# usnistgov/semantic-segmentation-unet

Hardware: AMD Instinct MI355X
Metric: training images/sec (higher is better)
Workload: dtype f32; 1 GPU; U-Net train step, synthetic 512x512x1, 2 classes, batch 8/GPU, f32 (BASELINE config 2); global_batch=8, parallelism=dp1, measured=2/bf16x6: 236.5 img/s

## Files before the change

include/unet_hip.h:

```cpp
#ifndef UNET_HIP_H
#define UNET_HIP_H
#include <stddef.h>
#include <stdint.h>
#ifdef __cplusplus
extern "C" {
#endif

#define UNET_OK 0
#define UNET_EINVAL (-1)
#define UNET_ENOSPC (-2)

#define UNET_HIP_ABI_VERSION 9
int unet_hip_abi_version(void);

int unet_conv3x3_mfma_supported(int Cin, int Cout);
int unet_conv3x3_fwd_mfma(const float* x, int ldx, const float* w, const float* bias, float* out, int ldo,
                          int N, int H, int W, int Cin, int Cout, int relu, void* stream);
int unet_conv3x3_dgrad_mfma(const float* dz, int lddz, const float* w, float* dx, int lddx,
                            int N, int H, int W, int Cin, int Cout, void* stream);
size_t unet_conv3x3_wgrad_mfma_workspace(int N, int H, int W, int Cin, int Cout);
int unet_conv3x3_wgrad_mfma(const float* xin, int ldx, const float* dz, int lddz, float* dw,
                            int N, int H, int W, int Cin, int Cout, void* ws, size_t ws_bytes, void* stream);
int unet_winograd_weight_transform(const float* w, float* U, int Cin, int Cout, int mode, void* stream);
int unet_winograd_weight_transform_batch(const void* jobs, int njobs, int total_blocks, void* stream);
// ... 81 lines not shown
int unet_convT2x2_wgrad_x6(const float* xin, int ldx, const float* dz, int lddz, float* dw,
                           int N, int H, int W, int Cin, int Cout, void* ws, size_t ws_bytes, void* stream);
size_t unet_convT2x2_wgrad_workspace(int N, int H, int W, int Cin, int Cout);
int unet_convT2x2_wgrad(const float* xin, int ldx, const float* dz, int lddz, float* dw,
                        int N, int H, int W, int Cin, int Cout, void* ws, size_t ws_bytes, void* stream);

int unet_bf16_pack_weights_batch(const void* jobs, int njobs, int total_blocks, void* stream);
int unet_convT2x2_bf16_supported(int N, int H, int W, int Cin, int Cout);
size_t unet_convT2x2_bf16_packed_bytes(int Cin, int Cout);
int unet_convT2x2_bf16_pack_weights(const float* w, void* packed, int Cin, int Cout, int mode, void* stream);
int unet_convT2x2_bf16_stats_rows(int N, int H, int W, int Cin, int Cout, int dgrad);
int unet_convT2x2_fwd_bf16(const void* x, int ldx, int x_bf16, const void* wp, const float* bias, void* out, int ldo, int out_bf16,
                           int N, int H, int W, int Cin, int Cout, float* stat_part, size_t stat_bytes, void* stream);
int unet_convT2x2_dgrad_bf16(const void* dz, int lddz, int dz_bf16, const void* wpd, void* dx, int lddx, int dx_bf16,
                             int N, int H, int W, int Cin, int Cout, const void* r_prev, int ldr, int r_bf16,
                             float* stat_part, size_t stat_bytes, void* stream);
int unet_convT2x2_wgrad_bf16_supported(int N, int H, int W, int Cin, int Cout);
size_t unet_convT2x2_wgrad_bf16_workspace(int N, int H, int W, int Cin, int Cout);
int unet_convT2x2_wgrad_bf16(const void* xin, int ldx, int x_bf16, const void* dz, int lddz, int dz_bf16, float* dw,
                                int N, int H, int W, int Cin, int Cout, void* ws, size_t ws_bytes, void* stream);

size_t unet_bn_workspace(long P, int C);
int unet_bn_train_stats(const float* r, int ldr, long P, int C, const float* gamma, const float* beta,
                        float eps, float momentum, int unbiased_moving_var, float* moving_mean, float* moving_var,
                        float* mean, float* invstd, float* scale, float* shift, void* ws, size_t ws_bytes, void* stream);
int unet_bn_train_finalize_partials(const float* part, int rows, long P, int C, const float* gamma, const float* beta,
                                    float eps, float momentum, int unbiased_moving_var, float* moving_mean, float* moving_var,
                                    float* mean, float* invstd, float* scale, float* shift, void* stream);
int unet_bn_eval_coeffs(const float* gamma, const float* beta, const float* moving_mean, const float* moving_var,
                        float eps, int C, float* scale, float* shift, void* stream);
int unet_bn_apply(const float* r, int ldr, const float* scale, const float* shift, float* y, int ldy, long P, int C, void* stream);
int unet_bn_apply_maxpool(const float* r, int ldr, const float* scale, const float* shift, float* y, int ldy,
                          float* pooled, int ldp, uint8_t* idx, int N, int H, int W, int C, void* stream);
int unet_bn_bwd(const float* dy, int lddy, const float* r, int ldr, const float* gamma, const float* mean,
                const float* invstd, long P, int C, int relu, float* dz, int lddz, float* dgamma, float* dbeta,
                float* dbias, void* ws, size_t ws_bytes, void* stream);

int unet_bn_bwd_pooled(const float* dy_skip, int lddy, const float* pooled_dy, int ldp, const uint8_t* idx, int N, int H, int W,
                       const float* r, int ldr, const float* gamma, const float* mean, const float* invstd, int C, int relu,
                       float* dz, int lddz, float* dgamma, float* dbeta, float* dbias, void* ws, size_t ws_bytes, void* stream);
int unet_bn_bwd_any(const void* dy, int lddy, const void* pooled_dy, int ldp, const uint8_t* idx, int N, int H, int W,
                    const void* r, int ldr, const float* gamma, const float* mean, const float* invstd, int C, int relu,
                    void* dz, int lddz, int dz_bf16, float* dgamma, float* dbeta, float* dbias, const float* part_sums, int rows,
                    void* ws, size_t ws_bytes, void* stream, int r_bf16, int dy_bf16, int pooled_dy_bf16, int* host_bias_rows);
int unet_bn_bwd_bias(const void* ws, int rows, int C, float* dbias, void* stream);
int unet_bn_apply_any(const void* r, int ldr, int r_bf16, const float* scale, const float* shift, void* y, int ldy, int y_bf16,
                      void* pooled, int ldp, uint8_t* idx, int N, int H, int W, int C, void* stream);
int unet_bn_finalize_apply_any(const float* part, int rows, const float* gamma, const float* beta, float eps, float momentum,
                               int unbiased_moving_var, float* moving_mean, float* moving_var, float* mean, float* invstd,
                               uint32_t* counter, uint32_t counter_target,
                               const void* r, int ldr, int r_bf16, float* scale, float* shift, void* y, int ldy, int y_bf16,
                               void* pooled, int ldp, uint8_t* idx, int N, int H, int W, int C, void* stream);
int unet_bn_bwd_from_partials(const float* dy, int lddy, const float* r, int ldr, const float* gamma, const float* mean,
                              const float* invstd, long P, int C, int relu, float* dz, int lddz, float* dgamma, float* dbeta,
                              float* dbias, const float* part_sums, int rows, void* ws, size_t ws_bytes, void* stream);

int unet_maxpool2x2_fwd(const void* x, int ldx, void* y, int ldy, uint8_t* idx, int N, int H, int W, int C, int t_bf16, void* stream);
int unet_maxpool2x2_bwd(const void* dy, int lddy, const uint8_t* idx, void* dx, int lddx,
                        int N, int H, int W, int C, int accumulate, int t_bf16, void* stream);
int unet_dropout(const void* x, int ldx, void* out, int ldo, long P, int C, const uint8_t* mask,
                 uint32_t seed, float rate, int t_bf16, void* stream);

size_t unet_softmax_ce_workspace(long P);
int unet_softmax_ce(const float* logits, int ldz, const int* labels_onehot, float* prob, float* dlogits, int lddz,
                    long P, int K, float label_smoothing, float loss_scale, float grad_scale, float ce_clip_eps,
                    float* loss_out, float* correct_out, void* ws, size_t ws_bytes, void* stream);
// ... 70 lines not shown
```

semantic-segmentation-unet_amd/csrc/norm.hip:

```cpp
#include "common.h"
#include <stdlib.h>

namespace {

typedef int i32x4v __attribute__((ext_vector_type(4)));
constexpr int kApplyNT = (UNET_NT & UNET_NT_LDAPPLY) != 0;

template <class T, int NT> __device__ __forceinline__ T bn_ld(const T* p) {
    if constexpr (NT != 0) return __builtin_nontemporal_load(p); else return *p;
}
template <int VEC, int NT = 0> __device__ __forceinline__ void vload(float (&v)[VEC], const float* p) {
    if constexpr (VEC == 8) {
        const f32x4 t = bn_ld<f32x4, NT>(reinterpret_cast<const f32x4*>(p)), u = bn_ld<f32x4, NT>(reinterpret_cast<const f32x4*>(p + 4));
        v[0] = t[0]; v[1] = t[1]; v[2] = t[2]; v[3] = t[3]; v[4] = u[0]; v[5] = u[1]; v[6] = u[2]; v[7] = u[3];
    } else if constexpr (VEC == 4) { const f32x4 t = bn_ld<f32x4, NT>(reinterpret_cast<const f32x4*>(p)); v[0] = t[0]; v[1] = t[1]; v[2] = t[2]; v[3] = t[3]; }
    else v[0] = *p;
}
__device__ __forceinline__ float bf_lo(unsigned w) { return __builtin_bit_cast(float, w << 16); }
__device__ __forceinline__ float bf_hi(unsigned w) { return __builtin_bit_cast(float, w & 0xffff0000u); }
template <int VEC, int NT = 0> __device__ __forceinline__ void vload_dt(float (&v)[VEC], const float* base, size_t idx, int in16) {
    if constexpr (VEC == 8) {
        if (in16) {
            const unet_u32x4 t = bn_ld<unet_u32x4, NT>(reinterpret_cast<const unet_u32x4*>(reinterpret_cast<const uint16_t*>(base) + idx));
            v[0] = bf_lo(t[0]); v[1] = bf_hi(t[0]); v[2] = bf_lo(t[1]); v[3] = bf_hi(t[1]);
// ... 282 lines not shown
        for (int e = 0; e < VEC; ++e) v[e] = fmaf(a[e], v[e], b[e]);
        vstore_dt<VEC>(y, (size_t)pix * ldy + c0, v, out16 & 1);
    }
}

template <int VEC>
__global__ __launch_bounds__(256) void bn_apply_pool_kernel(const float* __restrict__ r, int ldr, const float* scale,
        const float* shift, float* __restrict__ y, int ldy, float* __restrict__ pooled, int ldp, uint8_t* __restrict__ idx,
        int N, int H, int W, int C, int tpp, int out16, BnFin fin) {
    if (fin.part) bn_finalize_then_wait(fin, C, const_cast<float*>(scale), const_cast<float*>(shift));
    const Lay l = make_lay<VEC>(C, tpp);
    if (!l.active) return;
    const int H2 = H / 2, W2 = W / 2;
    const long total = (long)N * H2 * W2, S = (long)gridDim.x * l.npl;
    float a[VEC], b[VEC];
    bn_coef_load<VEC>(a, scale + l.c0, fin.part != nullptr); bn_coef_load<VEC>(b, shift + l.c0, fin.part != nullptr);
    for (long opix = (long)blockIdx.x * l.npl + l.pl; opix < total; opix += S) {
        long t = opix; const int ox = (int)(t % W2); t /= W2; const int oy = (int)(t % H2); const int n = (int)(t / H2);
        float best[VEC]; uint8_t bi[VEC];
        float v[4][VEC];
#pragma unroll
        for (int pos = 0; pos < 4; ++pos) {
            const size_t pix = (size_t)((long)n * H + 2 * oy + (pos >> 1)) * W + 2 * ox + (pos & 1);
            vload_dt<VEC, kApplyNT>(v[pos], r, pix * ldr + l.c0, out16 & 2);
        }
#pragma unroll
        for (int pos = 0; pos < 4; ++pos) {
            const size_t pix = (size_t)((long)n * H + 2 * oy + (pos >> 1)) * W + 2 * ox + (pos & 1);
#pragma unroll
            for (int e = 0; e < VEC; ++e) {
                v[pos][e] = fmaf(a[e], v[pos][e], b[e]);
                if (pos == 0 || v[pos][e] > best[e]) { best[e] = v[pos][e]; bi[e] = (uint8_t)pos; }
            }
            vstore_dt<VEC>(y, pix * ldy + l.c0, v[pos], out16 & 1);
        }
        vstore_dt<VEC>(pooled, (size_t)opix * ldp + l.c0, best, out16 & 1);
        const uint32_t w0 = (uint32_t)bi[0] | ((uint32_t)bi[1] << 8) | ((uint32_t)bi[2] << 16) | ((uint32_t)bi[3] << 24);
        if constexpr (VEC == 8) {
            const uint32_t w1 = (uint32_t)bi[4] | ((uint32_t)bi[5] << 8) | ((uint32_t)bi[6] << 16) | ((uint32_t)bi[7] << 24);
            *reinterpret_cast<uint2*>(idx + (size_t)opix * C + l.c0) = make_uint2(w0, w1);
        } else {
            *reinterpret_cast<uint32_t*>(idx + (size_t)opix * C + l.c0) = w0;
        }
    }
}

template <int VEC>
__global__ __launch_bounds__(256) void bn_bwd_reduce_kernel(const float* __restrict__ dy, int lddy, const float* __restrict__ r,
        int ldr, const float* __restrict__ mean, const float* __restrict__ invstd, long P, int C, int tpp, long ppb,
        double* __restrict__ part, PoolGrad pg, int dt) {
    extern __shared__ __attribute__((aligned(16))) double sRd[];
    const Lay l = make_lay<VEC>(C, tpp);
    const long p0 = (long)blockIdx.x * ppb; long p1 = p0 + ppb; if (p1 > P) p1 = P;
    double acc[2][VEC];
#pragma unroll
    for (int e = 0; e < VEC; ++e) { acc[0][e] = 0.0; acc[1][e] = 0.0; }
    if (l.active) {
        float mu[VEC]; vload<VEC>(mu, mean + l.c0);
        long pix = p0 + l.pl;
        const long st = l.npl;
        for (; pix + 3 * st < p1; pix += 4 * st) {
            float g[4][VEC], v[4][VEC];
#pragma unroll
            for (int u = 0; u < 4; ++u) {
                vload_dt<VEC>(g[u], dy, (size_t)(pix + u * st) * lddy + l.c0, dt & 4); vload_dt<VEC>(v[u], r, (size_t)(pix + u * st) * ldr + l.c0, dt & 2);
                add_pool_grad<VEC>(g[u], pg, pix + u * st, l.c0);
            }
// ... 445 lines not shown
    pl->vec = vec; pl->tpp = tpp; pl->nblk = (int)nblk; pl->ppb = (P + nblk - 1) / nblk;
    pl->smem2 = (size_t)256 * vec * 2 * sizeof(double); pl->smem1 = (size_t)256 * vec * sizeof(double);
    return true;
}

int nblk_for(long P) { (void)P; return (int)MAX_BLOCKS; }

constexpr bool bn_wide_always() { return true; }

int bn_cus() {
    static int cus = 0;
    if (!cus) { int dev = 0; hipDeviceProp_t pr; (void)hipGetDevice(&dev); cus = (hipGetDeviceProperties(&pr, dev) == hipSuccess && pr.multiProcessorCount > 0) ? pr.multiProcessorCount : 256; }
    return cus;
}

template <class K> int resident_grid(K kernel, size_t smem) {
    int per_cu = 0;
    if (hipOccupancyMaxActiveBlocksPerMultiprocessor(&per_cu, kernel, 256, smem) != hipSuccess || per_cu < 1) per_cu = 4;
    long g = (long)per_cu * bn_cus();
    return (int)(g > MAX_BLOCKS ? MAX_BLOCKS / bn_cus() * bn_cus() : g);
}
template <int VEC> int reduce_grid(size_t smem) { static int g = 0; if (!g) g = resident_grid(bn_bwd_reduce_kernel<VEC>, smem); return g; }
template <int VEC> int apply_grid(size_t smem) { static int g = 0; if (!g) g = resident_grid(bn_bwd_apply_kernel<VEC>, smem); return g; }
int pool16_grid(int which, size_t smem) {
    static int g[2] = {0, 0};
    if (!g[which]) g[which] = which ? resident_grid(bn_bwd_apply_pool16_kernel, smem) : resident_grid(bn_bwd_reduce_pool16_kernel, smem);
    return g[which];
}
int apply16_grid(size_t smem) { static int g = 0; if (!g) g = resident_grid(bn_bwd_apply16_kernel, smem); return g; }

int launch_bn_apply(const float* r, int ldr, int r16, const float* scale, const float* shift, float* y, int ldy, int y16,
                    float* pooled, int ldp, uint8_t* idx, int N, int H, int W, int C, hipStream_t st, const BnFin* finp = nullptr) {
    BnFin fin{}; if (finp) fin = *finp;
    const int flags = (y16 ? 1 : 0) | (r16 ? 2 : 0);
    const long P = (long)N * H * W;
    const bool al = unet_aligned16(r) && unet_aligned16(y) && unet_aligned16(scale) && unet_aligned16(shift) && (!pooled || unet_aligned16(pooled));
    int vec = 1;
    if ((flags || bn_wide_always()) && al && C % 8 == 0 && ldr % 8 == 0 && ldy % 8 == 0 && (!pooled || ldp % 8 == 0) && 256 % (C / 8) == 0) vec = 8;
    else if (al && C % 4 == 0 && ldr % 4 == 0 && ldy % 4 == 0 && (!pooled || ldp % 4 == 0)) vec = 4;
    if (flags && vec < 4) return UNET_EINVAL;
    int tpp = C / vec;
    bool lanes = (256 % tpp == 0);
    if (vec == 1) { tpp = 1; while (tpp < C) tpp <<= 1; lanes = tpp <= 256; }
    if (pooled) {
        if (!lanes || vec < 4) return UNET_EINVAL;
        const long total = (long)N * (H / 2) * (W / 2), npl = 256 / tpp;
        long blocks = (total + npl * 2 - 1) / (npl * 2); if (blocks > MAX_BLOCKS) blocks = MAX_BLOCKS; if (blocks < 1) blocks = 1;
        if (vec == 8) bn_apply_pool_kernel<8><<<(int)blocks, 256, 0, st>>>(r, ldr, scale, shift, y, ldy, pooled, ldp, idx, N, H, W, C, tpp, flags, fin);
        else          bn_apply_pool_kernel<4><<<(int)blocks, 256, 0, st>>>(r, ldr, scale, shift, y, ldy, pooled, ldp, idx, N, H, W, C, tpp, flags, fin);
        return UNET_LAUNCH_STATUS();
    }
    if (lanes) {
        const long npl = 256 / tpp;
        long blocks = (P + npl * 4 - 1) / (npl * 4); if (blocks > MAX_BLOCKS) blocks = MAX_BLOCKS; if (blocks < 1) blocks = 1;
        if (vec == 8)      bn_apply_kernel<8><<<(int)blocks, 256, 0, st>>>(r, ldr, scale, shift, y, ldy, P, C, tpp, flags, fin);
        else if (vec == 4) bn_apply_kernel<4><<<(int)blocks, 256, 0, st>>>(r, ldr, scale, shift, y, ldy, P, C, tpp, flags, fin);
        else               bn_apply_kernel<1><<<(int)blocks, 256, 0, st>>>(r, ldr, scale, shift, y, ldy, P, C, tpp, flags, fin);
    } else {
        if (fin.part) return UNET_EINVAL;
        const long total = P * (C / vec);
        long blocks = (total + 255) / 256; if (blocks > 8192) blocks = 8192;
        if (vec == 8)      bn_apply_flat_kernel<8><<<(int)blocks, 256, 0, st>>>(r, ldr, scale, shift, y, ldy, P, C, flags);
        else if (vec == 4) bn_apply_flat_kernel<4><<<(int)blocks, 256, 0, st>>>(r, ldr, scale, shift, y, ldy, P, C, flags);
        else               bn_apply_flat_kernel<1><<<(int)blocks, 256, 0, st>>>(r, ldr, scale, shift, y, ldy, P, C, flags);
    }
    return UNET_LAUNCH_STATUS();
// ... 21 lines not shown
    return UNET_LAUNCH_STATUS();
}

extern "C" int unet_bn_train_finalize_partials(const float* part, int rows, long P, int C, const float* gamma, const float* beta,
        float eps, float momentum, int unbiased_moving_var, float* moving_mean, float* moving_var,
        float* mean, float* invstd, float* scale, float* shift, void* stream) {
    UNET_CHECK_ARG(part && rows > 0 && P > 0 && C > 0 && C % 64 == 0 && gamma && beta && mean && invstd && scale && shift);
    UNET_CHECK_ARG((moving_mean == nullptr) == (moving_var == nullptr));
    bn_train_finalize_partials_kernel<<<C, 256, 0, (hipStream_t)stream>>>(part, rows, P, C, gamma, beta, eps, momentum,
        unbiased_moving_var, moving_mean, moving_var, mean, invstd, scale, shift);
    return UNET_LAUNCH_STATUS();
}

extern "C" int unet_bn_eval_coeffs(const float* gamma, const float* beta, const float* moving_mean, const float* moving_var,
                                   float eps, int C, float* scale, float* shift, void* stream) {
    UNET_CHECK_ARG(gamma && beta && moving_mean && moving_var && scale && shift && C > 0);
    bn_eval_coeffs_kernel<<<unet_cdiv(C, 128), 128, 0, (hipStream_t)stream>>>(gamma, beta, moving_mean, moving_var, eps, C, scale, shift);
    return UNET_LAUNCH_STATUS();
}

extern "C" int unet_bn_apply(const float* r, int ldr, const float* scale, const float* shift, float* y, int ldy,
                             long P, int C, void* stream) {
    UNET_CHECK_ARG(r && scale && shift && y && P > 0 && P < ((long)1 << 31) && C > 0 && ldr >= C && ldy >= C);
    return launch_bn_apply(r, ldr, 0, scale, shift, y, ldy, 0, nullptr, 0, nullptr, 1, 1, (int)P, C, (hipStream_t)stream);
}

extern "C" int unet_bn_apply_maxpool(const float* r, int ldr, const float* scale, const float* shift, float* y, int ldy,
                                     float* pooled, int ldp, uint8_t* idx, int N, int H, int W, int C, void* stream) {
    UNET_CHECK_ARG(r && scale && shift && y && pooled && idx && N > 0 && H > 0 && W > 0 && H % 2 == 0 && W % 2 == 0 && C > 0 && C % 4 == 0);
    UNET_CHECK_ARG(ldr >= C && ldy >= C && ldp >= C && ldr % 4 == 0 && ldy % 4 == 0 && ldp % 4 == 0);
    UNET_CHECK_ARG(unet_aligned16(r) && unet_aligned16(y) && unet_aligned16(pooled) && unet_aligned16(scale) && unet_aligned16(shift) &&
                   (reinterpret_cast<uintptr_t>(idx) & 3u) == 0);
    return launch_bn_apply(r, ldr, 0, scale, shift, y, ldy, 0, pooled, ldp, idx, N, H, W, C, (hipStream_t)stream);
}

static int bn_bwd_launch(const float* dy, int lddy, const float* r, int ldr, const float* gamma, const float* mean,
        const float* invstd, long P, int C, int relu, float* dz, int lddz, float* dgamma, float* dbeta, float* dbias,
        const float* part_sums, int rows, PoolGrad pg, void* ws, size_t ws_bytes, void* stream, int dt = 0, int* host_bias_rows = nullptr) {
    UNET_CHECK_ARG(dy && r && gamma && mean && invstd && dz && dgamma && dbeta && (dbias || host_bias_rows) && ws && P > 0 && C > 0);
    UNET_CHECK_ARG(lddy >= C && ldr >= C && lddz >= C);
    Plan pl;
    const bool al = unet_aligned16(dy) && unet_aligned16(r) && unet_aligned16(dz) && unet_aligned16(gamma) && unet_aligned16(mean) &&
                    unet_aligned16(invstd) && unet_aligned16(dgamma) && unet_aligned16(dbeta) && (!pg.pdy || (unet_aligned16(pg.pdy) && pg.ldp % 4 == 0));
    UNET_CHECK_ARG(make_plan(P, C, lddy, ldr, lddz, al && (!pg.pdy || pg.ldp % 8 == 0 || !(dt || pg.p16)), &pl, dt != 0 || pg.p16 != 0 || bn_wide_always()));
    if (ws_bytes < unet_bn_workspace(P, C)) return UNET_ENOSPC;
    hipStream_t st = (hipStream_t)stream;
    double* part = (double*)ws;
    int rc;
    if ((dt || pg.p16) && pl.vec < 4) return UNET_EINVAL;
    int nb_r = pl.nblk, nb_a = pl.nblk;
    {
        const int cr = pl.vec == 8 ? reduce_grid<8>(pl.smem2) : pl.vec == 4 ? reduce_grid<4>(pl.smem2) : reduce_grid<1>(pl.smem2);
        const int ca = pl.vec == 8 ? apply_grid<8>(pl.smem1) : pl.vec == 4 ? apply_grid<4>(pl.smem1) : apply_grid<1>(pl.smem1);
        if (nb_r > cr) nb_r = cr;
        if (nb_a > ca) nb_a = ca;
    }
    const bool pooled_form = pg.pdy != nullptr && pl.vec >= 4;
    const long Pw = pooled_form ? P / 4 : P;
    if (pooled_form) {
        const long npl = 256 / pl.tpp;
        long nb = (Pw + npl * 4 - 1) / (npl * 4); if (nb < 1) nb = 1;
        if (nb_r > nb) nb_r = (int)nb;
        if (nb_a > nb) nb_a = (int)nb;
    }
    const size_t ldmax = (size_t)(lddy > ldr ? (lddy > lddz ? lddy : lddz) : (ldr > lddz ? ldr : lddz));
    const bool small16 = (size_t)P * ldmax * 2 < ((size_t)1 << 31);
// ... 122 lines not shown
```

semantic-segmentation-unet_amd/engine.py:

```python
import ctypes
import math

import numpy as np
import torch

from ._lib import lib
from .plan import BF16, EngineOptions, PRODUCER, build_plan, layer_table

BASE = 64
SIZE_FACTOR = 16

BN_EPS = 1e-3
BN_MOMENTUM = 0.99
BN_MOVING_VAR_UNBIASED = 1
DROPOUT_RATE = 0.5
ADAM_BETA1, ADAM_BETA2, ADAM_EPS = 0.9, 0.999, 1e-7
CE_CLIP_EPS = 0.0


def kernel_shape(kind, cin, cout):
    return {"conv3": (3, 3, cin, cout), "conv1": (1, 1, cin, cout), "deconv": (2, 2, cout, cin)}[kind]


BACKWARD_ORDER = ["logits", "dec_1b", "dec_1a", "up_1", "dec_2b", "dec_2a", "up_2", "dec_3b", "dec_3a", "up_3",
# ... 35 lines not shown
        if self.dev.type != "cuda":
            raise RuntimeError("the U-Net hot path runs on an MI355X only (device must be cuda); no CPU fallback exists")
        self.L = lib()
        self.opt = options if options is not None else EngineOptions.from_env()
        self._plans = {}
        self.pl = None
        self.layers = layer_table(number_channels, number_classes)
        self.kind = {n: k for n, k, _, _ in self.layers}
        self.cin = {n: ci for n, _, ci, _ in self.layers}
        self.cout = {n: co for n, _, _, co in self.layers}
        self.slices, self.layer_range, off = flat_layout(number_channels, number_classes)
        self.n_flat = off
        self.theta = torch.zeros(off, dtype=torch.float32, device=self.dev)
        self.grad = torch.zeros_like(self.theta)
        self.adam_m = torch.zeros_like(self.theta)
        self.adam_v = torch.zeros_like(self.theta)
        self.p = {k: self.theta[o:o + n].view(shape) for k, (o, n, shape) in self.slices.items()}
        self.g = {k: self.grad[o:o + n].view(shape) for k, (o, n, shape) in self.slices.items()}
        self.moving = {}
        self.stat = {}
        for name, _, _, co in self.layers:
            self.moving[name + "/moving_mean"] = torch.zeros(co, dtype=torch.float32, device=self.dev)
            self.moving[name + "/moving_var"] = torch.ones(co, dtype=torch.float32, device=self.dev)
            cp = (co + 3) // 4 * 4
            self.stat[name] = torch.zeros(4, cp, dtype=torch.float32, device=self.dev)
        self.iterations = 0
        self.bufs = {}
        self._ws = None
        self.loss_buf = torch.zeros(2, dtype=torch.float32, device=self.dev)
        self.dropout_seed = seed
        self.ce_clip_eps = CE_CLIP_EPS
        self._eval_folded = set()
        self._eval_coefs = set()
        self.view = {}
        self._fused_U, self._fused_dirty = None, True
        self._x6_U, self._x6_dirty = None, True
        self._ctx6_W, self._ctx6_dirty = None, True
        self._bf16_W, self._bf16_dirty = {}, True
        self.bnbwd_part = {}
        self.init_parameters(seed)
        self.on_layer_grads_ready = None
        self.profile = None
        self.side = torch.cuda.Stream(device=self.dev)
        self._ws_side = None

    @property
    def compute_dtype(self):
        return self.opt.compute_dtype

    @compute_dtype.setter
    def compute_dtype(self, v):
        if v not in ("fp32", "bf16"):
            raise ValueError("compute_dtype must be 'fp32' or 'bf16'")
        self.opt.compute_dtype = v

    @property
    def overlap_wgrad(self):
        return self.opt.overlap_wgrad

    @overlap_wgrad.setter
    def overlap_wgrad(self, v):
        self.opt.overlap_wgrad = bool(v)

    def plan(self, n, h, w, training=False, want_grad=False):
        key = (n, h, w, bool(training), bool(want_grad), self.opt.key())
        pl = self._plans.get(key)
# ... 165 lines not shown
        t = self.bufs.get(name)
        if t is None or tuple(t.shape) != tuple(shape) or t.dtype != dtype:
            t = torch.empty(shape, dtype=dtype, device=self.dev)
            self.bufs[name] = t
        return t

    def _workspace(self, nbytes, side=False):
        cur = self._ws_side if side else self._ws
        if cur is None or cur.numel() < nbytes:
            cur = torch.empty(int(nbytes) + 256, dtype=torch.uint8, device=self.dev)
            if side:
                self._ws_side = cur
            else:
                self._ws = cur
        return cur

    @staticmethod
    def _stream():
        return ctypes.c_void_p(torch.cuda.current_stream().cuda_stream)

    def _fold_buffers(self, name, x6=False):
        cin, cout = self.cin[name], self.cout[name]
        if x6:
            return (self._buf("U6fold_" + name, (self.L.unet_winograd_x6_weight_bytes(cin, cout),), torch.uint8),
                    self._buf("bfold_" + name, (cout,)), self._buf("pad_" + name, (cin + 8,)))
        return (self._buf("Ufold_" + name, (16 * cin * cout,)), self._buf("bfold_" + name, (cout,)), self._buf("pad_" + name, (cin + 8,)))

    def _block_fwd(self, name, x, y_out, training, pool=None, in_view=None, r_out=None, stat_out=None):
        L, st = self.L, self._stream()
        cap = self.opt.cap
        lp = self.pl.layer[name]
        kind, cin, cout = lp.kind, lp.cin, lp.cout
        n, h, w, _ = x.shape
        assert (h, w) == (lp.hi, lp.wi) and (in_view is not None) == lp.x_on_load and (y_out is None) == lp.defer_y, name
        w_, b_ = self.p[name + "/kernel"], self.p[name + "/bias"]
        fused_stats = None
        r16 = lp.r == BF16
        assert not (r16 and r_out is not None)
        if r_out is not None:
            r = r_out
        else:
            r = self._buf(("r16_" if r16 else "r_") + name, (n, lp.ho, lp.wo, cout), torch.bfloat16 if r16 else torch.float32)
        part = lambda rows: self._buf("bnpart_" + name, ((cout // 64) * rows * 128,)) if rows > 0 else None
        if lp.fwd == "convt_bf16":
            rows = L.unet_convT2x2_bf16_stats_rows(n, h, w, cin, cout, 0) if lp.fwd_stats else 0
            stat_part = part(rows)
            self._timed("convt_fwd_bf16", 8.0 * n * h * w * cin * cout, L.unet_convT2x2_fwd_bf16,
                        _p(x), _ld(x), int(x.dtype == torch.bfloat16), _p(self._bf16_kernels(name)[0]), _p(b_), _p(r), _ld(r),
                        int(r16), n, h, w, cin, cout, _p(stat_part), stat_part.numel() * 4 if rows > 0 else 0, st)
            fused_stats = (stat_part, rows) if rows > 0 else None
        elif lp.fwd == "convt_x6":
            rows = L.unet_convT2x2_x6_stats_rows(n, h, w, cin, cout) if lp.fwd_stats else 0
            stat_part = part(rows)
            self._timed("convt_fwd_x6", 8.0 * n * h * w * cin * cout, L.unet_convT2x2_fwd_x6,
                        _p(x), _ld(x), _p(self._convt_x6_kernels(name)[0]), _p(b_), _p(r), _ld(r), n, h, w, cin, cout,
                        _p(stat_part), stat_part.numel() * 4 if rows > 0 else 0, st)
            fused_stats = (stat_part, rows) if rows > 0 else None
        elif lp.fwd == "convt_stream" and _ld(x) <= 4096:
            rows = L.unet_convT2x2_fwd_stream_stats_rows_wg(n, h, w, cin, cout, cap) if lp.fwd_stats else 0
            stat_part = part(rows)
            self._timed("convt_fwd", 8.0 * n * h * w * cin * cout, L.unet_convT2x2_fwd_stream_wg,
                        _p(x), _ld(x), _p(w_), _p(b_), _p(r), _ld(r), n, h, w, cin, cout,
                        _p(stat_part), stat_part.numel() * 4 if rows > 0 else 0, cap, st)
            fused_stats = (stat_part, rows) if rows > 0 else None
        elif kind == "deconv":
            L.unet_convT2x2_fwd(_p(x), _ld(x), _p(w_), _p(b_), _p(r), _ld(r), n, h, w, cin, cout, st)
        elif kind == "conv1":
# ... 51 lines not shown
        mm, mv = self.moving[name + "/moving_mean"], self.moving[name + "/moving_var"]
        merged = training and fused_stats is not None and self.opt.merge_bn_finalize and y_out is not None and cout % 64 == 0
        if merged:
            cnt = self._fin_counters()
            i = self._fin_index[name]
            self._fin_target[i] = (self._fin_target[i] + cout) & 0xFFFFFFFF
            self._timed("bn_apply", self._nb(r, y_out, *(pool or ())), L.unet_bn_finalize_apply_any,
                        _p(fused_stats[0]), fused_stats[1], _p(gm), _p(bt), BN_EPS, BN_MOMENTUM, BN_MOVING_VAR_UNBIASED, _p(mm), _p(mv), _p(s[0]), _p(s[1]),
                        ctypes.c_void_p(cnt.data_ptr() + 4 * i), self._fin_target[i],
                        _p(r), _ld(r), int(r.dtype == torch.bfloat16), _p(sc_out), _p(sh_out), _p(y_out), _ld(y_out), int(y_out.dtype == torch.bfloat16),
                        _p(pool[0]) if pool is not None else None, cout, _p(pool[1]) if pool is not None else None,
                        r.shape[0], r.shape[1], r.shape[2], cout, st)
            self._eval_coefs.clear()
            self.saved[name] = (x, r)
            self.view[name] = in_view
            self.coef[name] = (sc_out, sh_out)
            return y_out
        if training and fused_stats is not None:
            L.unet_bn_train_finalize_partials(_p(fused_stats[0]), fused_stats[1], P, cout, _p(gm), _p(bt), BN_EPS, BN_MOMENTUM,
                                              BN_MOVING_VAR_UNBIASED, _p(mm), _p(mv), _p(s[0]), _p(s[1]), _p(sc_out), _p(sh_out), st)
        elif training:
            nb = L.unet_bn_workspace(P, cout)
            ws = self._workspace(nb)
            self._timed("bn_stats", self._nb(r), L.unet_bn_train_stats, _p(r), _ld(r), P, cout, _p(gm), _p(bt), BN_EPS, BN_MOMENTUM,
                        BN_MOVING_VAR_UNBIASED, _p(mm), _p(mv), _p(s[0]), _p(s[1]), _p(sc_out), _p(sh_out), _p(ws), nb, st)
        elif (name, sc_out.data_ptr()) not in self._eval_coefs:
            L.unet_bn_eval_coeffs(_p(gm), _p(bt), _p(mm), _p(mv), BN_EPS, cout, _p(sc_out), _p(sh_out), st)
            self._eval_coefs.add((name, sc_out.data_ptr()))
        if training:
            self._eval_coefs.clear()
        self.saved[name] = (x, r)
        self.view[name] = in_view
        self.coef[name] = (sc_out, sh_out)
        if y_out is None:
            return r
        if r.dtype == torch.bfloat16 or y_out.dtype == torch.bfloat16:
            self._timed("bn_apply", self._nb(r, y_out, *(pool or ())), L.unet_bn_apply_any,
                        _p(r), _ld(r), int(r.dtype == torch.bfloat16), _p(sc_out), _p(sh_out), _p(y_out), _ld(y_out), int(y_out.dtype == torch.bfloat16),
                        _p(pool[0]) if pool is not None else None, cout, _p(pool[1]) if pool is not None else None,
                        r.shape[0], r.shape[1], r.shape[2], cout, st)
        elif pool is not None:
            self._timed("bn_apply", self._nb(r, y_out, *pool), L.unet_bn_apply_maxpool,
                        _p(r), _ld(r), _p(sc_out), _p(sh_out), _p(y_out), _ld(y_out), _p(pool[0]), cout, _p(pool[1]),
                        r.shape[0], r.shape[1], r.shape[2], cout, st)
        else:
            self._timed("bn_apply", self._nb(r, y_out), L.unet_bn_apply, _p(r), _ld(r), _p(sc_out), _p(sh_out), _p(y_out), _ld(y_out), P, cout, st)
        return y_out

    def _dropout(self, t, key, masks, backward=False):
        n, h, w, c = t.shape
        m = None
        if masks is not None:
            m = masks[key]
        seed = (self.dropout_seed * 1000003 + self.iterations * 2 + (0 if key == "drop_4" else 1)) & 0xFFFFFFFF
        self._timed("dropout", 2 * self._nb(t), self.L.unet_dropout,
                    _p(t), _ld(t), _p(t), _ld(t), n * h * w, c, _p(m), seed, DROPOUT_RATE, int(t.dtype == torch.bfloat16), self._stream())

    def _prep_masks(self, dropout_masks):
        if dropout_masks is None:
            return None
        out = {}
        for k, v in dropout_masks.items():
            a = np.ascontiguousarray(np.asarray(v).transpose(0, 2, 3, 1)).astype(np.uint8)
            out[k] = torch.as_tensor(a).to(self.dev)
        return out

    def forward(self, images, training=False, dropout_masks=None, labels=None, global_batch_size=None,
                label_smoothing=0.0, want_grad=False):
        L, st = self.L, self._stream()
        x = images
        assert x.dtype == torch.float32 and x.dim() == 4 and x.shape[1] == self.C, "images must be fp32 [N,C,H,W]"
        x = x.to(self.dev).contiguous()
        n, c, h, w = x.shape
        if h % SIZE_FACTOR or w % SIZE_FACTOR:
            raise IOError("Input Image tile size must be a multiple of %d" % SIZE_FACTOR)
        if c == 1:
            x0 = x.view(n, h, w, 1)
        else:
            x0 = self._buf("x_nhwc", (n, h, w, c))
            L.unet_nchw_to_nhwc(_p(x), _p(x0), n, c, h, w, st)
# ... 2 lines not shown
        self.coef = {}
        self.masks = self._prep_masks(dropout_masks) if training else None
        pl = self.pl = self.plan(n, h, w, training, want_grad)
        if training:
            self._eval_folded.clear()
        B = BASE
        f = self._block_fwd
        tdt = lambda d: torch.bfloat16 if d == BF16 else torch.float32
        cur, cur_view = x0, None
        self.idx = {}
        self.cat = {}
        self.catstat = {}

        def ybuf(name, shape):
            d = pl.layer[name].y
            return self._buf(("y16_" if d == BF16 else "y_") + name, shape, tdt(d))

        def pair(a_name, b_name, xin, xin_view, hh, ww, ch, b_out, **kw):
            if pl.layer[a_name].defer_y:
                ra = f(a_name, xin, None, training, in_view=xin_view)
                sa = self.stat[a_name]
                return f(b_name, ra, b_out, training, in_view=(sa[2], sa[3]), **kw)
            ya = f(a_name, xin, ybuf(a_name, (n, hh, ww, ch)), training, in_view=xin_view)
            return f(b_name, ya, b_out, training, **kw)

        for lvl, ch in ((1, B), (2, 2 * B), (3, 4 * B), (4, 8 * B)):
            hh, ww = cur.shape[1], cur.shape[2]
            c16 = pl.cat[lvl] == BF16
            cat = self._buf(("cat16_%d" if c16 else "cat_%d") % lvl, (n, hh, ww, 2 * ch), tdt(pl.cat[lvl]))
            self.cat[lvl] = cat
            pooled = self._buf(("pool16_%d" if c16 else "pool_%d") % lvl, (n, hh // 2, ww // 2, ch), tdt(pl.cat[lvl]))
            idx = self._buf("idx_%d" % lvl, (n, hh // 2, ww // 2, ch), torch.uint8)
            fuse_pool = pl.fuse_pool[lvl]
            skip = pair("conv_%da" % lvl, "conv_%db" % lvl, cur, cur_view, hh, ww, ch, cat[..., :ch], pool=(pooled, idx) if fuse_pool else None)
            if not fuse_pool:
                if lvl == 4 and training:
                    self._dropout(skip, "drop_4", self.masks)
                assert skip.dtype == pooled.dtype
                self._timed("pool", self._nb(skip, pooled, idx), L.unet_maxpool2x2_fwd,
                            _p(skip), _ld(skip), _p(pooled), ch, _p(idx), n, hh, ww, ch, int(skip.dtype == torch.bfloat16), st)
            self.idx[lvl] = idx
            cur, cur_view = pooled, None
        hh, ww = cur.shape[1], cur.shape[2]
        cur = pair("bott_a", "bott_b", cur, None, hh, ww, 16 * B, ybuf("bott_b", (n, hh, ww, 16 * B)))
        if training:
            self._dropout(cur, "drop_b", self.masks)
        for lvl, ch in ((4, 8 * B), (3, 4 * B), (2, 2 * B), (1, B)):
            cat = self.cat[lvl]
            hh, ww = cat.shape[1], cat.shape[2]
            cat_view = None
            if pl.layer["up_%d" % lvl].defer_y:
                cs = self.bufs.get("catstat_%d" % lvl)
                if cs is None:
                    cs = self._buf("catstat_%d" % lvl, (2, 2 * ch))
                    cs[0, :ch].fill_(1.0); cs[1, :ch].zero_()
                self.catstat[lvl] = cs
                f("up_%d" % lvl, cur, None, training, r_out=cat[..., ch:], stat_out=(cs[0, ch:], cs[1, ch:]))
                cat_view = (cs[0], cs[1])
            else:
                f("up_%d" % lvl, cur, cat[..., ch:], training)
            cur = pair("dec_%da" % lvl, "dec_%db" % lvl, cat, cat_view, hh, ww, ch, ybuf("dec_%db" % lvl, (n, hh, ww, ch)))
        yl = f("logits", cur, self._buf("y_logits", (n, h, w, self.K)), training)
        prob = self._buf("softmax", (n, h, w, self.K))
        P = n * h * w
        nb = L.unet_softmax_ce_workspace(P)
        ws = self._workspace(nb)
        if labels is None:
            L.unet_softmax_ce(_p(yl), self.K, None, _p(prob), None, 0, P, self.K, 0.0, 0.0, 0.0, 0.0, None, None, _p(ws), nb, st)
        else:
            lab = labels.to(self.dev).contiguous()
            assert lab.dtype == torch.int32 and tuple(lab.shape) == (n, h, w, self.K), "labels must be int32 one-hot [N,H,W,K]"
            G = global_batch_size if global_batch_size else n
            scale = 1.0 / (float(G) * h * w)
            dl = self._buf("dy_logits", (n, h, w, self.K)) if want_grad else None
            self._timed("softmax_ce", self._nb(yl, lab, prob, dl), L.unet_softmax_ce,
                        _p(yl), self.K, _p(lab), _p(prob), _p(dl), self.K, P, self.K, float(label_smoothing), scale,
                        scale, float(self.ce_clip_eps), _p(self.loss_buf[0:1]), _p(self.loss_buf[1:2]), _p(ws), nb, st)
            self._labels_keepalive = lab
        return prob

    def _block_bwd(self, name, dy, eval_mode=False, pool_grad=None):
        L, st = self.L, self._stream()
        lp = self.pl.layer[name]
        kind, cin, cout = lp.kind, lp.cin, lp.cout
        x, r = self.saved[name]
        n, ho, wo, _ = r.shape
        P = n * ho * wo
        s = self.stat[name]
        dz16 = lp.dz == BF16
# ... 195 lines not shown
```

semantic-segmentation-unet_amd/plan.py:

```python
import dataclasses
import os
from dataclasses import dataclass, field
from typing import Dict, Optional, Tuple

BASE = 64

F32, BF16 = "f32", "bf16"


@dataclass
class EngineOptions:
    compute_dtype: str = "fp32"
    conv_route: str = "fused"
    fp32_matrix: str = "bf16x6"
    wgrad_route: str = "fused"
    bn_on_load: bool = True
    fuse_bn_stats: bool = True
    fuse_pool: bool = True
    merge_bn_finalize: bool = False
    bf16_storage: bool = True
    bf16_activations: bool = True
    overlap_wgrad: bool = True
    max_workgroups: Optional[int] = None

    @staticmethod
    def from_env(env=None):
        env = os.environ if env is None else env
        o = EngineOptions()
        o.compute_dtype = env.get("UNET_COMPUTE_DTYPE", o.compute_dtype)
        o.conv_route = env.get("UNET_CONV_ROUTE", o.conv_route)
        o.wgrad_route = env.get("UNET_WGRAD_ROUTE", o.wgrad_route)
        o.fp32_matrix = env.get("UNET_FP32_MATRIX", o.fp32_matrix)
        for name, var in (("bn_on_load", "UNET_BN_ON_LOAD"), ("fuse_bn_stats", "UNET_FUSE_BN_STATS"), ("fuse_pool", "UNET_FUSE_POOL"),
                          ("merge_bn_finalize", "UNET_MERGE_BN_FINALIZE"), ("bf16_storage", "UNET_BF16_STORAGE"), ("bf16_activations", "UNET_BF16_ACTIVATIONS"),
                          ("overlap_wgrad", "UNET_OVERLAP_WGRAD")):
            if var in env:
                setattr(o, name, env[var] != "0")
        if "UNET_MAX_WORKGROUPS" in env:
            o.max_workgroups = int(env["UNET_MAX_WORKGROUPS"])
        if o.compute_dtype not in ("fp32", "bf16"):
            raise ValueError("compute_dtype must be 'fp32' or 'bf16'")
        if o.fp32_matrix not in ("bf16x6", "native"):
            raise ValueError("fp32_matrix must be 'bf16x6' or 'native'")
        return o

    def key(self):
        return dataclasses.astuple(self)

    @property
    def cap(self):
        return int(self.max_workgroups or 0)


PRODUCER = {"bott_b": ("bott_a", 0, 1, 1)}
for _l in (1, 2, 3, 4):
    PRODUCER["conv_%db" % _l] = ("conv_%da" % _l, 0, 1, 1)
    PRODUCER["dec_%db" % _l] = ("dec_%da" % _l, 0, 1, 1)
    PRODUCER["dec_%da" % _l] = ("up_%d" % _l, 1, 2, 2)
for _l in (1, 2, 3):
    PRODUCER["up_%d" % _l] = ("dec_%db" % (_l + 1), 0, 1, 1)

CONSUMER = {"bott_a": "bott_b", "bott_b": "up_4", "dec_1b": "logits"}
for _l in (1, 2, 3, 4):
    CONSUMER["conv_%da" % _l] = "conv_%db" % _l
    CONSUMER["dec_%da" % _l] = "dec_%db" % _l
    CONSUMER["up_%d" % _l] = "dec_%da" % _l
for _l in (2, 3, 4):
    CONSUMER["dec_%db" % _l] = "up_%d" % (_l - 1)


@dataclass
class LayerPlan:
    name: str
    kind: str
    cin: int
    cout: int
    hi: int
    wi: int
    ho: int
    wo: int
    fwd: str = ""
    dgrad: str = ""
    wgrad: str = ""
    fwd_x6: bool = False
    dgrad_x6: bool = False
    x_on_load: bool = False
    defer_y: bool = False
    r: str = F32
    y: Optional[str] = F32
    dz: str = F32
    dx: Optional[str] = F32
    fwd_stats: bool = False
    sums_from_dgrad: bool = False
    leaves_sums_for: Optional[Tuple[str, int, int]] = None


@dataclass
class StepPlan:
    n: int
    h: int
    w: int
    training: bool
    want_grad: bool
    options: Tuple
    layer: Dict[str, LayerPlan] = field(default_factory=dict)
    cat: Dict[int, str] = field(default_factory=dict)
    fuse_pool: Dict[int, bool] = field(default_factory=dict)
    lvl4_grad: str = F32

    def describe(self):
        rows = ["plan n=%d h=%d w=%d training=%s want_grad=%s" % (self.n, self.h, self.w, self.training, self.want_grad)]
        for p in self.layer.values():
            rows.append("%-8s %-6s %4d->%-4d @%dx%d  fwd=%-12s dgrad=%-11s wgrad=%-10s r=%s y=%s dz=%s dx=%s%s%s%s%s" % (
                p.name, p.kind, p.cin, p.cout, p.ho, p.wo, p.fwd + ("/x6" if p.fwd_x6 else ""), p.dgrad + ("/x6" if p.dgrad_x6 else ""), p.wgrad, p.r, p.y, p.dz, p.dx,
                " on_load" if p.x_on_load else "", " defer_y" if p.defer_y else "", " fwd_stats" if p.fwd_stats else "",
                " sums<-" + CONSUMER.get(p.name, "?") if p.sums_from_dgrad else ""))
        rows.append("concat/pool storage: " + " ".join("L%d=%s%s" % (l, d, "(fused)" if self.fuse_pool[l] else "") for l, d in self.cat.items()))
        return "\n".join(rows)

    def rounding_points(self):
        L = self.layer
        return dict(
            contract=frozenset(n for n, p in L.items() if p.fwd in ("bf16", "convt_bf16") and p.wgrad in ("bf16", "convt_bf16")),
            r_bf16=frozenset(n for n, p in L.items() if p.r == BF16),
            y_bf16=frozenset(n for n, p in L.items() if p.y == BF16 and n in CONSUMER and L[CONSUMER[n]].fwd not in ("bf16", "convt_bf16")),
            dz_bf16=frozenset(n for n, p in L.items() if p.dz == BF16),
            dx_bf16=frozenset(n for n, p in L.items() if p.dx == BF16),
            sums_from_dgrad=frozenset(n for n, p in L.items() if p.sums_from_dgrad),
            lvl4_accumulate_bf16=self.lvl4_grad == BF16)


def layer_table(number_channels, number_classes):
    C, K, B = number_channels, number_classes, BASE
    return [
        ("conv_1a", "conv3", C, B), ("conv_1b", "conv3", B, B),
        ("conv_2a", "conv3", B, 2 * B), ("conv_2b", "conv3", 2 * B, 2 * B),
        ("conv_3a", "conv3", 2 * B, 4 * B), ("conv_3b", "conv3", 4 * B, 4 * B),
        ("conv_4a", "conv3", 4 * B, 8 * B), ("conv_4b", "conv3", 8 * B, 8 * B),
        ("bott_a", "conv3", 8 * B, 16 * B), ("bott_b", "conv3", 16 * B, 16 * B),
        ("up_4", "deconv", 16 * B, 8 * B), ("dec_4a", "conv3", 16 * B, 8 * B), ("dec_4b", "conv3", 8 * B, 8 * B),
        ("up_3", "deconv", 8 * B, 4 * B), ("dec_3a", "conv3", 8 * B, 4 * B), ("dec_3b", "conv3", 4 * B, 4 * B),
        ("up_2", "deconv", 4 * B, 2 * B), ("dec_2a", "conv3", 4 * B, 2 * B), ("dec_2b", "conv3", 2 * B, 2 * B),
        ("up_1", "deconv", 2 * B, B), ("dec_1a", "conv3", 2 * B, B), ("dec_1b", "conv3", B, B),
        ("logits", "conv1", B, K),
    ]


def _level(name):
# ... 79 lines not shown
    st2 = bf and opt.bf16_storage
    st3 = st2 and opt.bf16_activations
    for p in pl.layer.values():
        if train and st2 and allbf(p.name) and (p.dgrad in ("bf16", "convt_bf16")):
            p.dz = BF16
        if train and st3 and p.fwd_stats and p.dz == BF16:
            p.r = BF16
    if train and st3 and first.fwd == "direct" and first.fwd_stats and first.cout % 8 == 0:
        first.r = first.dz = BF16
    for name, p in pl.layer.items():
        cons = CONSUMER.get(name)
        if cons is not None and cons != "logits" and st2 and allbf(cons):
            p.y = BF16
    if train and want_grad and st3:
        pl.layer["dec_1b"].y = BF16
    for lvl in (1, 2, 3, 4):
        nxt = "conv_%da" % (lvl + 1) if lvl < 4 else "bott_a"
        pl.fuse_pool[lvl] = opt.fuse_pool and not (lvl == 4 and train)
        c16 = st2 and opt.fuse_pool and (lvl < 4 or st3) and allbf("dec_%da" % lvl) and allbf(nxt)
        pl.cat[lvl] = BF16 if c16 else F32
        pl.layer["conv_%db" % lvl].y = pl.cat[lvl]
        pl.layer["up_%d" % lvl].y = pl.cat[lvl]

    def can_defer(a, b):
        pb = pl.layer[b]
        return (opt.bn_on_load and not bf and opt.wgrad_route == "fused" and pb.fwd == "winograd" and pb.wgrad == "winograd"
                and pl.layer[a].y == F32)
    for lvl in (1, 2, 3, 4):
        for a, b in (("conv_%da" % lvl, "conv_%db" % lvl), ("dec_%da" % lvl, "dec_%db" % lvl), ("up_%d" % lvl, "dec_%da" % lvl)):
            if can_defer(a, b):
                pl.layer[a].defer_y, pl.layer[a].y, pl.layer[b].x_on_load = True, None, True
    if can_defer("bott_a", "bott_b"):
        pl.layer["bott_a"].defer_y, pl.layer["bott_a"].y, pl.layer["bott_b"].x_on_load = True, None, True

    if train:
        for name, p in pl.layer.items():
            prod = PRODUCER.get(name)
            if prod is None or not opt.fuse_bn_stats or p.dgrad == "none":
                continue
            pp = pl.layer[prod[0]]
            ok = False
            if p.dgrad == "bf16":
                ok = L.unet_conv3x3_bf16_stats_rows(n, p.ho, p.wo, p.cout, p.cin) > 0
            elif p.dgrad == "winograd":
                ok = pp.r == F32 and L.unet_conv3x3_fwd_winograd_fused_stats_rows_wg(n, p.ho, p.wo, p.cout, p.cin, opt.cap) > 0
            elif p.dgrad == "convt_bf16":
                ok = L.unet_convT2x2_bf16_stats_rows(n, p.hi, p.wi, p.cin, p.cout, 1) > 0
            elif p.dgrad == "convt_x6":
                ok = pp.r == F32 and L.unet_convT2x2_x6_bnbwd_rows(n, p.hi, p.wi, p.cin, p.cout) > 0
            if ok:
                c0, c1 = prod[1] * (p.cin // prod[3]), prod[2] * (p.cin // prod[3])
                p.leaves_sums_for = (prod[0], c0, c1)
                pp.sums_from_dgrad = True

        takes16 = lambda nm: pl.layer[nm].dz == BF16
        d4 = (st3 and pl.layer["dec_4a"].dgrad == "bf16" and pl.layer["bott_a"].dgrad == "bf16" and pl.cat[4] == BF16)
        pl.lvl4_grad = BF16 if d4 else F32
        for name, p in pl.layer.items():
            if not st3 or p.dx is None:
                continue
            ok = False
            if p.kind == "conv1":
                ok = p.cin % 8 == 0 and takes16("dec_1b")
            elif p.kind == "deconv":
                ok = p.dgrad == "convt_bf16" and p.leaves_sums_for is not None and takes16(p.leaves_sums_for[0])
            elif p.dgrad == "bf16":
# ... 21 lines not shown
```

Before: 236.1 images/sec.

## Apply BN-ReLU to encoder skip tensors on load instead of materializing them

For encoder levels 1-3, conv_Xb now stores only the raw pre-BN output into the concat buffer, and its BN-apply kernel writes just the pooled output and indices, skipping the full-resolution normalized skip write. The decoder's concat consumer normalizes the skip half on load using per-channel scale/shift stored in catstat. This removes a full-resolution f32 write (and later read) per level. It adds coupling between the encoder plan and the decoder's on-load path, plus cache invalidation of the eval coefficients when the mode changes.

```diff
diff --git a/include/unet_hip.h b/include/unet_hip.h
--- a/include/unet_hip.h
+++ b/include/unet_hip.h
@@ -137,6 +137,8 @@
 int unet_bn_apply(const float* r, int ldr, const float* scale, const float* shift, float* y, int ldy, long P, int C, void* stream);
 int unet_bn_apply_maxpool(const float* r, int ldr, const float* scale, const float* shift, float* y, int ldy,
                           float* pooled, int ldp, uint8_t* idx, int N, int H, int W, int C, void* stream);
+int unet_bn_apply_pool_only(const float* r, int ldr, const float* scale, const float* shift,
+                            float* pooled, int ldp, uint8_t* idx, int N, int H, int W, int C, void* stream);
 int unet_bn_bwd(const float* dy, int lddy, const float* r, int ldr, const float* gamma, const float* mean,
                 const float* invstd, long P, int C, int relu, float* dz, int lddz, float* dgamma, float* dbeta,
                 float* dbias, void* ws, size_t ws_bytes, void* stream);
diff --git a/semantic-segmentation-unet_amd/csrc/norm.hip b/semantic-segmentation-unet_amd/csrc/norm.hip
--- a/semantic-segmentation-unet_amd/csrc/norm.hip
+++ b/semantic-segmentation-unet_amd/csrc/norm.hip
@@ -338,7 +338,7 @@
                 v[pos][e] = fmaf(a[e], v[pos][e], b[e]);
                 if (pos == 0 || v[pos][e] > best[e]) { best[e] = v[pos][e]; bi[e] = (uint8_t)pos; }
             }
-            vstore_dt<VEC>(y, pix * ldy + l.c0, v[pos], out16 & 1);
+            if (y) vstore_dt<VEC>(y, pix * ldy + l.c0, v[pos], out16 & 1);
         }
         vstore_dt<VEC>(pooled, (size_t)opix * ldp + l.c0, best, out16 & 1);
         const uint32_t w0 = (uint32_t)bi[0] | ((uint32_t)bi[1] << 8) | ((uint32_t)bi[2] << 16) | ((uint32_t)bi[3] << 24);
@@ -850,6 +850,7 @@
 int launch_bn_apply(const float* r, int ldr, int r16, const float* scale, const float* shift, float* y, int ldy, int y16,
                     float* pooled, int ldp, uint8_t* idx, int N, int H, int W, int C, hipStream_t st, const BnFin* finp = nullptr) {
     BnFin fin{}; if (finp) fin = *finp;
+    if (!y && !pooled) return UNET_EINVAL;
     const int flags = (y16 ? 1 : 0) | (r16 ? 2 : 0);
     const long P = (long)N * H * W;
     const bool al = unet_aligned16(r) && unet_aligned16(y) && unet_aligned16(scale) && unet_aligned16(shift) && (!pooled || unet_aligned16(pooled));
@@ -937,6 +938,15 @@
     UNET_CHECK_ARG(unet_aligned16(r) && unet_aligned16(y) && unet_aligned16(pooled) && unet_aligned16(scale) && unet_aligned16(shift) &&
                    (reinterpret_cast<uintptr_t>(idx) & 3u) == 0);
     return launch_bn_apply(r, ldr, 0, scale, shift, y, ldy, 0, pooled, ldp, idx, N, H, W, C, (hipStream_t)stream);
+}
+
+extern "C" int unet_bn_apply_pool_only(const float* r, int ldr, const float* scale, const float* shift,
+                                       float* pooled, int ldp, uint8_t* idx, int N, int H, int W, int C, void* stream) {
+    UNET_CHECK_ARG(r && scale && shift && pooled && idx && N > 0 && H > 0 && W > 0 && H % 2 == 0 && W % 2 == 0 && C > 0 && C % 4 == 0);
+    UNET_CHECK_ARG(ldr >= C && ldp >= C && ldr % 4 == 0 && ldp % 4 == 0);
+    UNET_CHECK_ARG(unet_aligned16(r) && unet_aligned16(pooled) && unet_aligned16(scale) && unet_aligned16(shift) &&
+                   (reinterpret_cast<uintptr_t>(idx) & 7u) == 0);
+    return launch_bn_apply(r, ldr, 0, scale, shift, nullptr, 0, 0, pooled, ldp, idx, N, H, W, C, (hipStream_t)stream);
 }
 
 static int bn_bwd_launch(const float* dy, int lddy, const float* r, int ldr, const float* gamma, const float* mean,
diff --git a/semantic-segmentation-unet_amd/engine.py b/semantic-segmentation-unet_amd/engine.py
--- a/semantic-segmentation-unet_amd/engine.py
+++ b/semantic-segmentation-unet_amd/engine.py
@@ -91,6 +91,7 @@
         self.ce_clip_eps = CE_CLIP_EPS
         self._eval_folded = set()
         self._eval_coefs = set()
+        self._catstat_skip = {}
         self.view = {}
         self._fused_U, self._fused_dirty = None, True
         self._x6_U, self._x6_dirty = None, True
@@ -322,7 +323,8 @@
         lp = self.pl.layer[name]
         kind, cin, cout = lp.kind, lp.cin, lp.cout
         n, h, w, _ = x.shape
-        assert (h, w) == (lp.hi, lp.wi) and (in_view is not None) == lp.x_on_load and (y_out is None) == lp.defer_y, name
+        assert (h, w) == (lp.hi, lp.wi) and (in_view is not None) == lp.x_on_load and (y_out is None) == (lp.defer_y or lp.pool_only), name
+        assert not lp.pool_only or (pool is not None and r_out is not None and stat_out is not None), name
         w_, b_ = self.p[name + "/kernel"], self.p[name + "/bias"]
         fused_stats = None
         r16 = lp.r == BF16
@@ -440,6 +442,10 @@
         self.saved[name] = (x, r)
         self.view[name] = in_view
         self.coef[name] = (sc_out, sh_out)
+        if y_out is None and pool is not None:
+            self._timed("bn_apply", self._nb(r, *pool), L.unet_bn_apply_pool_only,
+                        _p(r), _ld(r), _p(sc_out), _p(sh_out), _p(pool[0]), cout, _p(pool[1]), r.shape[0], r.shape[1], r.shape[2], cout, st)
+            return r
         if y_out is None:
             return r
         if r.dtype == torch.bfloat16 or y_out.dtype == torch.bfloat16:
@@ -454,6 +460,17 @@
         else:
             self._timed("bn_apply", self._nb(r, y_out), L.unet_bn_apply, _p(r), _ld(r), _p(sc_out), _p(sh_out), _p(y_out), _ld(y_out), P, cout, st)
         return y_out
+
+    def _catstat(self, lvl, ch, skip_on_load):
+        cs = self._buf("catstat_%d" % lvl, (2, 2 * ch))
+        was = self._catstat_skip.get(lvl)
+        if was is not None and was != skip_on_load:
+            self._eval_folded.clear(); self._eval_coefs.clear()
+        if not skip_on_load and was is not False:
+            cs[0, :ch].fill_(1.0); cs[1, :ch].zero_()
+        self._catstat_skip[lvl] = skip_on_load
+        self.catstat[lvl] = cs
+        return cs
 
     def _dropout(self, t, key, masks, backward=False):
         n, h, w, c = t.shape
@@ -522,7 +539,12 @@
             pooled = self._buf(("pool16_%d" if c16 else "pool_%d") % lvl, (n, hh // 2, ww // 2, ch), tdt(pl.cat[lvl]))
             idx = self._buf("idx_%d" % lvl, (n, hh // 2, ww // 2, ch), torch.uint8)
             fuse_pool = pl.fuse_pool[lvl]
-            skip = pair("conv_%da" % lvl, "conv_%db" % lvl, cur, cur_view, hh, ww, ch, cat[..., :ch], pool=(pooled, idx) if fuse_pool else None)
+            if pl.layer["conv_%db" % lvl].pool_only:
+                cs = self._catstat(lvl, ch, True)
+                skip = pair("conv_%da" % lvl, "conv_%db" % lvl, cur, cur_view, hh, ww, ch, None, pool=(pooled, idx),
+                            r_out=cat[..., :ch], stat_out=(cs[0, :ch], cs[1, :ch]))
+            else:
+                skip = pair("conv_%da" % lvl, "conv_%db" % lvl, cur, cur_view, hh, ww, ch, cat[..., :ch], pool=(pooled, idx) if fuse_pool else None)
             if not fuse_pool:
                 if lvl == 4 and training:
                     self._dropout(skip, "drop_4", self.masks)
@@ -540,11 +562,7 @@
             hh, ww = cat.shape[1], cat.shape[2]
             cat_view = None
             if pl.layer["up_%d" % lvl].defer_y:
-                cs = self.bufs.get("catstat_%d" % lvl)
-                if cs is None:
-                    cs = self._buf("catstat_%d" % lvl, (2, 2 * ch))
-                    cs[0, :ch].fill_(1.0); cs[1, :ch].zero_()
-                self.catstat[lvl] = cs
+                cs = self._catstat(lvl, ch, lvl < 4 and pl.layer["conv_%db" % lvl].pool_only)
                 f("up_%d" % lvl, cur, None, training, r_out=cat[..., ch:], stat_out=(cs[0, ch:], cs[1, ch:]))
                 cat_view = (cs[0], cs[1])
             else:
diff --git a/semantic-segmentation-unet_amd/plan.py b/semantic-segmentation-unet_amd/plan.py
--- a/semantic-segmentation-unet_amd/plan.py
+++ b/semantic-segmentation-unet_amd/plan.py
@@ -15,6 +15,7 @@
     fp32_matrix: str = "bf16x6"
     wgrad_route: str = "fused"
     bn_on_load: bool = True
+    skip_on_load: bool = True
     fuse_bn_stats: bool = True
     fuse_pool: bool = True
     merge_bn_finalize: bool = False
@@ -31,7 +32,7 @@
         o.conv_route = env.get("UNET_CONV_ROUTE", o.conv_route)
         o.wgrad_route = env.get("UNET_WGRAD_ROUTE", o.wgrad_route)
         o.fp32_matrix = env.get("UNET_FP32_MATRIX", o.fp32_matrix)
-        for name, var in (("bn_on_load", "UNET_BN_ON_LOAD"), ("fuse_bn_stats", "UNET_FUSE_BN_STATS"), ("fuse_pool", "UNET_FUSE_POOL"),
+        for name, var in (("bn_on_load", "UNET_BN_ON_LOAD"), ("skip_on_load", "UNET_SKIP_ON_LOAD"), ("fuse_bn_stats", "UNET_FUSE_BN_STATS"), ("fuse_pool", "UNET_FUSE_POOL"),
                           ("merge_bn_finalize", "UNET_MERGE_BN_FINALIZE"), ("bf16_storage", "UNET_BF16_STORAGE"), ("bf16_activations", "UNET_BF16_ACTIVATIONS"),
                           ("overlap_wgrad", "UNET_OVERLAP_WGRAD")):
             if var in env:
@@ -86,6 +87,7 @@
     dgrad_x6: bool = False
     x_on_load: bool = False
     defer_y: bool = False
+    pool_only: bool = False
     r: str = F32
     y: Optional[str] = F32
     dz: str = F32
@@ -111,9 +113,9 @@
     def describe(self):
         rows = ["plan n=%d h=%d w=%d training=%s want_grad=%s" % (self.n, self.h, self.w, self.training, self.want_grad)]
         for p in self.layer.values():
-            rows.append("%-8s %-6s %4d->%-4d @%dx%d  fwd=%-12s dgrad=%-11s wgrad=%-10s r=%s y=%s dz=%s dx=%s%s%s%s%s" % (
+            rows.append("%-8s %-6s %4d->%-4d @%dx%d  fwd=%-12s dgrad=%-11s wgrad=%-10s r=%s y=%s dz=%s dx=%s%s%s%s%s%s" % (
                 p.name, p.kind, p.cin, p.cout, p.ho, p.wo, p.fwd + ("/x6" if p.fwd_x6 else ""), p.dgrad + ("/x6" if p.dgrad_x6 else ""), p.wgrad, p.r, p.y, p.dz, p.dx,
-                " on_load" if p.x_on_load else "", " defer_y" if p.defer_y else "", " fwd_stats" if p.fwd_stats else "",
+                " on_load" if p.x_on_load else "", " defer_y" if p.defer_y else "", " pool_only" if p.pool_only else "", " fwd_stats" if p.fwd_stats else "",
                 " sums<-" + CONSUMER.get(p.name, "?") if p.sums_from_dgrad else ""))
         rows.append("concat/pool storage: " + " ".join("L%d=%s%s" % (l, d, "(fused)" if self.fuse_pool[l] else "") for l, d in self.cat.items()))
         return "\n".join(rows)
@@ -259,6 +261,11 @@
                 pl.layer[a].defer_y, pl.layer[a].y, pl.layer[b].x_on_load = True, None, True
     if can_defer("bott_a", "bott_b"):
         pl.layer["bott_a"].defer_y, pl.layer["bott_a"].y, pl.layer["bott_b"].x_on_load = True, None, True
+    for lvl in (1, 2, 3):
+        pb = pl.layer["conv_%db" % lvl]
+        if (opt.skip_on_load and pl.fuse_pool[lvl] and pl.layer["up_%d" % lvl].defer_y and pl.cat[lvl] == F32 and pb.r == F32
+                and pb.cout % 4 == 0):
+            pb.pool_only = True
 
     if train:
         for name, p in pl.layer.items():
```

Result: no change. 237.4 images/sec, median of 4 (+0.6%).
